# tlemane/kmtricks

Measured on AMD Instinct MI355X. Metric: k-mers merged/s (merge stage, sum over partitions of input records / time), higher is better.
Workload: dtype u64 keys / u32 counts (integer)

## Files before the change

kmtricks_amd/csrc/kmx_api.hip:

```cpp
#include "kmx_host.hpp"

#include <algorithm>
#include <chrono>
#include <cmath>
#include <sys/mman.h>
#include <unordered_map>
#include <mutex>
#include <cstdlib>
#include <cstring>
#include <memory>

using namespace kmx;

static thread_local std::string g_create_err;

void* kmx_ctx::dalloc(size_t bytes)
{
  if (bytes == 0) bytes = 256;
  if (bytes >= (8u << 20)) { size_t p2 = (size_t)1 << 23; while (p2 * 2 <= bytes) p2 *= 2; const size_t q = p2 >> 3; bytes = (bytes + q - 1) / q * q; }
  int best = -1;
  for (size_t i = 0; i < pool.size(); i++)
    if (!pool[i].used && pool[i].bytes >= bytes && pool[i].bytes <= 2 * bytes + (1u << 20) &&
        (best < 0 || pool[i].bytes < pool[best].bytes)) best = (int)i;
  if (best >= 0) { pool[best].used = true; return pool[best].p; }
// ... 494 lines not shown
      u32 rt_max = 0; bool rec_bits = true, any_share = false;
      for (auto& H : R->tasks) { rt_max = std::max(rt_max, H.rt); rec_bits = rec_bits && std::max(H.rec_min, H.share_min) <= 1u; any_share = any_share || H.share_min > 0; }
      const u32 bgrid = std::min(R->n_items, (u32)ctx->n_cu * 2u);
      static const bool two_walks_env = getenv("KMX_BFT_TWO_WALKS") != nullptr;
      if (rec_bits && any_share && !R->bft_two_walks && !two_walks_env && !R->d_rem) {
        u64 per_tile = 0;
        for (auto& H : R->tasks) { const u64 tiles = std::max<u64>(1, ((H.upper - H.lower + 1) + H.rt - 1) / H.rt); per_tile = std::max(per_tile, H.total_recs / tiles); }
        u64 cap = std::max<u64>(4096, per_tile / 4);
        cap = std::min<u64>(cap, ((1ull << 30) / 8) / std::max(1u, bgrid));
        R->rem_cap = (u32)cap;
        R->d_rem = (u64*)ctx->dalloc((size_t)bgrid * cap * 8);
      }
      const bool one_walk = R->d_rem && !R->bft_two_walks;
      bool wide = false;
      for (auto& H : R->tasks) { const double m = (double)H.total_recs / H.N * (double)H.rt / (double)(H.upper - H.lower + 1); wide = wide || m + 2.6 * std::sqrt(m) + 8 > (double)bft_round_records(false); }
      KMX_HIP(ctx, launch_merge_bft(d_tasks, d_items, R->n_items, d_ticket, bgrid, R->max_n, rt_max, rec_bits, wide, one_walk ? R->d_rem : nullptr, R->rem_cap, ctx->stream));
    } else
    KMX_HIP(ctx, launch_merge_bf(mode == KMX_MODE_BFC, d_tasks, d_items, R->n_items, d_ticket, R->grid, R->bf_lds, ctx->stream));
  } else if (R->use_cols) {
    const TaskDev* d_subs = reinterpret_cast<const TaskDev*>(R->d_meta + R->o_subtasks);
    const uint2* d_subitems = reinterpret_cast<const uint2*>(R->d_meta + R->o_subitems);
    const ColsDev* d_cols = reinterpret_cast<const ColsDev*>(R->d_meta + R->o_cols);
    const uint2* d_citems = reinterpret_cast<const uint2*>(R->d_meta + R->o_citems);
    static const bool overlap = getenv("KMX_COLS_PREP_OVERLAP") != nullptr;
    hipStream_t ps = overlap ? ctx->aux : ctx->stream;
    if (!R->ev_pre) KMX_HIP(ctx, hipEventCreateWithFlags(&R->ev_pre, hipEventDisableTiming));
    if (overlap && ctx->stream_shared) {
      KMX_HIP(ctx, hipEventRecord(R->ev_pre, ctx->stream));
      KMX_HIP(ctx, hipStreamWaitEvent(ctx->aux, R->ev_pre, 0));
    }
    if (!overlap) KMX_HIP(ctx, hipStreamWaitEvent(ctx->stream, R->ev_up, 0));
    KMX_HIP(ctx, launch_range_bounds(kw, d_subs, nt, R->sub_max_n, R->sub_max_c, ps));
    KMX_HIP(ctx, CO.skel(d_subs, d_subitems, R->n_subitems, ps));
    KMX_HIP(ctx, CO.prep(d_tasks, d_subs, d_cols, nt, ps));
    {
      u32 max_slots = 0;
      for (auto& H : R->tasks) max_slots = std::max(max_slots, H.slots_cap);
      const char* const tenv = getenv("KMX_COLS_SEED_TRIES");
      KMX_HIP(ctx, CO.seeds(d_tasks, d_cols, nt, max_slots, tenv && atoi(tenv) > 0 ? (u32)atoi(tenv) : 0u, getenv("KMX_TRACE") != nullptr, ps));
    }
    KMX_HIP(ctx, hipEventRecord(R->ev_pre, ps));
    KMX_HIP(ctx, hipStreamWaitEvent(ctx->stream, R->ev_up, 0));
    KMX_HIP(ctx, launch_range_bounds(kw, d_tasks, nt, R->max_n, R->max_c, ctx->stream));
    KMX_HIP(ctx, hipStreamWaitEvent(ctx->stream, R->ev_pre, 0));
    if (R->ev0) KMX_HIP(ctx, hipEventRecord(R->ev0, ctx->stream));
    const u32 cols_grid_env = getenv("KMX_COLS_GRID") ? (u32)atoi(getenv("KMX_COLS_GRID")) : 0u;
    const u32 sparse_cus_env = getenv("KMX_SPARSE_CUS") ? (u32)atoi(getenv("KMX_SPARSE_CUS")) : 0u;
    KMX_HIP(ctx, CO.merge(mode, (R->cols_ext ? 1 : 0) | (R->cols_resc ? 2 : 0) | (R->cols_ord ? 4 : 0) | (R->cols_narrow ? 8 : 0), d_tasks, d_cols, d_citems, R->n_citems, d_ticket,
                          cols_grid_env ? std::min(cols_grid_env, R->cols_grid) : R->cols_grid, ctx->stream));
    if (R->ev0) { if (!R->ev_mid) KMX_HIP(ctx, hipEventCreate(&R->ev_mid)); KMX_HIP(ctx, hipEventRecord(R->ev_mid, ctx->stream)); }
    KMX_HIP(ctx, CO.sparse(mode | (R->cols_resc ? 2 : 0) | (R->cols_ord ? 4 : 0), d_tasks, d_cols, d_items, R->n_items, nt, d_ticket, sparse_cus_env ? std::min(sparse_cus_env, (u32)ctx->n_cu) : (u32)ctx->n_cu, ctx->stream));
    if (R->share_fix) {
      if ((size_t)R->max_n * 4 > 48 * 1024) KMX_HIP(ctx, hipFuncSetAttribute(reinterpret_cast<const void*>(&k_share_fix), hipFuncAttributeMaxDynamicSharedMemorySize, (int)std::min<size_t>((size_t)R->max_n * 4, 160 * 1024)));
      hipLaunchKernelGGL(k_share_fix, dim3((unsigned)ctx->n_cu * 2u, nt), dim3(256), (size_t)R->max_n * 4, ctx->stream, (const TaskDev*)d_tasks, kw);
      KMX_HIP(ctx, hipGetLastError());
    }
    if (R->ev0) KMX_HIP(ctx, hipEventRecord(R->ev1, ctx->stream));
    return mirror_and_mark(R);
  } else {
    if (with_bounds) KMX_HIP(ctx, launch_range_bounds(kw, d_tasks, nt, R->max_n, R->max_c, ctx->stream));
    if (R->ev0) KMX_HIP(ctx, hipEventRecord(R->ev0, ctx->stream));
    if (R->use_pivot) KMX_HIP(ctx, launch_merge_pivot(kw, mode, d_tasks, d_items, R->n_items, d_ticket, R->grid, ctx->stream));
    else if (R->rows_small) KMX_HIP(ctx, launch_merge_rows_s(kw, mode, d_tasks, d_items, R->n_items, d_ticket, R->grid, R->max_n, ctx->stream));
    else KMX_HIP(ctx, launch_merge_rows(kw, mode, d_tasks, d_items, R->n_items, d_ticket, R->grid, R->max_n, ctx->stream));
  }
  if (R->ev0) KMX_HIP(ctx, hipEventRecord(R->ev1, ctx->stream));
  return mirror_and_mark(R);
}

__global__ __launch_bounds__(256)
void k_share_fix(const TaskDev* __restrict__ tasks, u32 kw)
{
  extern __shared__ u32 sm_s[];
  const TaskDev& T = tasks[blockIdx.y];
  if (T.mode != KMX_MODE_COUNT || T.share_min <= max(1u, T.rec_min)) return;
  if (T.ctrl[2] & (u64)(ERR_FALLBACK | ERR_ROWS_OVERFLOW)) return;
  const u64 rows = T.ctrl[0];
// ... 238 lines not shown
    max_n = std::max(max_n, H.N); max_c = std::max(max_c, H.c);
  }
  R->n_items = n_items; R->max_n = max_n; R->max_c = max_c;
  R->grid = std::min(n_items, is_bf ? slots : (u32)ctx->n_cu * (u32)(R->rows_small ? rows_s_wgs_per_cu((int)kw) : rows_wgs_per_cu((int)kw)));
  if (R->use_pivot) R->grid = std::min(n_items, (u32)ctx->n_cu);
  if (R->use_cols) {
    R->subs.resize(n_tasks);
    u32 nsub = 0, ncit = 0;
    for (u32 t = 0; t < n_tasks; t++) {
      const TaskHost& H = R->tasks[t];
      TaskHost& Q = R->subs[t];
      { const u32 S = cols_row_lists(std::max(1u, H.rec_min)); Q.N = std::min<u32>(S ? S : 32u, H.N); }
      Q.kw = kw; Q.mode = mode; Q.rec_min = H.rec_min; Q.share_min = 0;
      Q.len.resize(Q.N);
      u32 piv = 0;
      Q.src.resize(Q.N);
      std::vector<u32> win;
      for (u32 i = 0; i < Q.N; i++) {
        const u32 w0 = (u32)(((u64)i * H.N) / Q.N), w1 = std::max(w0 + 1, (u32)(((u64)(i + 1) * H.N) / Q.N));
        win.clear();
        for (u32 j = w0; j < w1; j++) win.push_back(j);
        std::nth_element(win.begin(), win.begin() + win.size() / 2, win.end(), [&](u32 a, u32 b) { return H.len[a] != H.len[b] ? H.len[a] < H.len[b] : a < b; });
        const u32 src = win[win.size() / 2];
        Q.src[i] = src;
        Q.len[i] = H.len[src]; Q.total_recs += H.len[src];
        if (Q.len[i] > Q.len[piv]) piv = i;
      }
      Q.pivot = (Q.N >= 2 && Q.len[Q.N / 2] > 0) ? Q.N / 2 : piv;
      Q.row_bytes = 8 * kw;
      u32 wl = 0; while (wl < 6 && (Q.N << (wl + 1)) <= (u32)rows_cap((int)kw, Q.N)) wl++;
      Q.wl = wl;
      Q.rows_guess = std::max<u64>(1, std::min<u64>(H.rows_guess, Q.total_recs));
      u64 c = std::min<u64>(2000, std::max<u64>(1, Q.total_recs / 1500));
      c = std::min<u64>(c, std::max<u32>(1, Q.len[Q.pivot]));
      Q.c = (u32)c;
      Q.seg_cap = Q.c;
      Q.out_cap_rows = (u64)Q.c * CO.skel_cap();
      Q.out_bytes = (size_t)(Q.out_cap_rows * Q.row_bytes);
      nsub += Q.c; ncit += H.c * H.nblk;
      R->sub_max_c = std::max(R->sub_max_c, Q.c); R->sub_max_n = std::max(R->sub_max_n, Q.N);
    }
    R->n_subitems = nsub; R->n_citems = ncit;
    R->sub_grid = std::min(nsub, (u32)ctx->n_cu * (u32)rows_wgs_per_cu((int)kw));
    R->cols_grid = std::min(ncit, cols_cus);
  }
  if (is_bf) {
    int lds = 0;
    for (auto& H : R->tasks) lds = std::max(lds, bf_lds_bytes(H.rt, H.row_bytes, H.N));
    R->bf_lds = lds;
  }

  for (auto& H : R->tasks) H.kernel = R->use_cols ? 2 : R->use_pivot ? 1 : 0;
  const bool cols = R->use_cols;
  size_t off = 0;
  R->o_tasks = off; off = align_up(off + sizeof(TaskDev) * n_tasks, 256);
  R->o_items = off; off = align_up(off + sizeof(uint2) * n_items, 256);
  R->o_ticket = off; off += 256;
  R->o_ctrl0 = off;
  for (auto& H : R->tasks) { H.o_ctrl = off; off += 64; }
  off = align_up(off, 256);
  auto lay_lists = [&](TaskHost& H) {
    H.o_recs = off; off = align_up(off + 8ull * H.N, 256);
    H.o_len = off; off = align_up(off + 4ull * H.N, 256);
    H.o_smin = off; off = align_up(off + 4ull * H.N, 256);
    H.o_stats = off; off = align_up(off + 8ull * 6 * H.N, 256);
  };
// ... 1193 lines not shown
```

kmtricks_amd/csrc/kmx_dev.hpp:

```cpp
#pragma once
#include <hip/hip_runtime.h>
#include <stdint.h>

namespace kmx {

typedef unsigned long long u64;
typedef uint32_t u32;
typedef uint16_t u16;
typedef uint8_t u8;
typedef __attribute__((address_space(1))) const u32 gu32;
struct __attribute__((packed, aligned(1))) UDword { u32 v; };
struct __attribute__((packed, aligned(1))) UShort { u16 v; };

struct Seg {
  u32 range;
  u32 seq;
  u64 row_off;
  u32 nrows;
  u32 pad;
};

struct TaskDev {
  const u8* const* recs;
  const u32* len;
// ... 49 lines not shown
#define KMX_CHUNK_BYTES 262144
#endif

enum { ERR_ROWS_OVERFLOW = 1, ERR_SEGS_OVERFLOW = 2, ERR_FALLBACK = 4,
       ERR_DIVERGENT = 8,
       ERR_SLICES = 16,
       ERR_DENSE_CAP = 32 };

template <int KW> struct Key { u64 w[KW]; };

template <int KW> __device__ __forceinline__ bool key_less(const Key<KW>& a, const Key<KW>& b) {
#pragma unroll
  for (int i = KW - 1; i > 0; i--) { if (a.w[i] != b.w[i]) return a.w[i] < b.w[i]; }
  return a.w[0] < b.w[0];
}
template <int KW> __device__ __forceinline__ bool key_eq(const Key<KW>& a, const Key<KW>& b) {
  bool e = a.w[0] == b.w[0];
#pragma unroll
  for (int i = 1; i < KW; i++) e = e && (a.w[i] == b.w[i]);
  return e;
}
template <int KW> __device__ __forceinline__ bool key_le(const Key<KW>& a, const Key<KW>& b) { return !key_less<KW>(b, a); }
template <int KW> __device__ __forceinline__ Key<KW> key_inf() { Key<KW> k; for (int i = 0; i < KW; i++) k.w[i] = ~0ULL; return k; }
template <int KW> __device__ __forceinline__ Key<KW> key_min(const Key<KW>& a, const Key<KW>& b) { return key_less<KW>(b, a) ? b : a; }

template <int KW> __device__ __forceinline__ Key<KW> load_key(const u8* p) {
  const u32* q = reinterpret_cast<const u32*>(p);
  Key<KW> k;
#pragma unroll
  for (int i = 0; i < KW; i++) k.w[i] = (u64)q[2 * i] | ((u64)q[2 * i + 1] << 32);
  return k;
}

template <int KW> __device__ __forceinline__ Key<KW> load_row_key(const u8* p) {
  if ((reinterpret_cast<uintptr_t>(p) & 3u) == 0) return load_key<KW>(p);
  Key<KW> k;
#pragma unroll
  for (int i = 0; i < KW; i++) {
    u64 w = 0;
#pragma unroll
    for (int b = 0; b < 8; b++) w |= (u64)p[8 * i + b] << (8 * b);
    k.w[i] = w;
  }
  return k;
}

__device__ __forceinline__ u64 shfl_xor_u64(u64 v, int m) {
  u32 lo = __shfl_xor((u32)v, m), hi = __shfl_xor((u32)(v >> 32), m);
  return (u64)lo | ((u64)hi << 32);
}
template <int KW> __device__ __forceinline__ Key<KW> wave_min_key(Key<KW> k) {
#pragma unroll
  for (int off = 32; off > 0; off >>= 1) {
    Key<KW> o;
#pragma unroll
    for (int i = 0; i < KW; i++) o.w[i] = shfl_xor_u64(k.w[i], off);
    k = key_min<KW>(k, o);
  }
  return k;
}
template <int M> __device__ __forceinline__ u32 xor_lane_u32(u32 v) {
  static_assert(M == 1 || M == 2 || M == 4 || M == 8 || M == 16 || M == 32, "a power of two below 64");
  if constexpr (M == 1) return (u32)__builtin_amdgcn_mov_dpp((int)v, 0xB1, 0xF, 0xF, true);
  else if constexpr (M == 2) return (u32)__builtin_amdgcn_mov_dpp((int)v, 0x4E, 0xF, 0xF, true);
  else if constexpr (M == 4)
    return (u32)__builtin_amdgcn_mov_dpp(__builtin_amdgcn_mov_dpp((int)v, 0x141, 0xF, 0xF, true), 0x1B, 0xF, 0xF, true);
// ... 13 lines not shown
```

kmtricks_amd/csrc/kmx_host.hpp:

```cpp
#pragma once
#include <hip/hip_runtime.h>
#include <string>
#include <functional>
#include <vector>
#include "kmx_dev.hpp"
#include "skf.hpp"
#include "../../include/kmx.h"

namespace kmx {

int rows_lds_bytes(int kw, u32 n_lists);
int rows_cap(int kw, u32 n_lists);
int rows_wgs_per_cu(int kw);
u32 rows_chunk_rows(u32 row_bytes);
u32 rows_image_bytes(int kw);
hipError_t launch_range_bounds(int kw, const TaskDev* tasks, u32 n_tasks, u32 max_n, u32 max_c, hipStream_t st);
hipError_t launch_merge_rows(int kw, int mode, const TaskDev* tasks, const uint2* items, u32 n_items, u32* ticket,
                             u32 grid_x, u32 max_n, hipStream_t st);
int rows_s_cap(int kw, u32 n_lists);
int rows_s_wgs_per_cu(int kw);
u32 rows_s_image_bytes(int kw);
hipError_t launch_merge_rows_s(int kw, int mode, const TaskDev* tasks, const uint2* items, u32 n_items, u32* ticket, u32 grid_x, u32 max_n, hipStream_t st);
int pivot_lds_bytes(int kw);
u32 pivot_max_lists();
hipError_t launch_merge_pivot(int kw, int mode, const TaskDev* tasks, const uint2* items, u32 n_items, u32* ticket,
                              u32 grid_x, hipStream_t st);
struct ColsOps {
  int (*lds_bytes)();
  u32 (*block_lists)();
  u32 (*wgs_per_cu)();
  u32 (*tile_rows)(u32 nb);
  u64 (*scratch_keys)(u32 slots, u32 nblk);
  u64 (*scratch_counts)(u32 slots, u32 nblk);
  u64 (*ext_entries)(u32 slots, u32 nblk);
  u32 (*skel_cap)();
  hipError_t (*skel)(const TaskDev* subs, const uint2* items, u32 n_items, hipStream_t st);
  hipError_t (*prep)(const TaskDev* tasks, const TaskDev* subs, const ColsDev* cols, u32 n_tasks, hipStream_t st);
  hipError_t (*seeds)(const TaskDev* tasks, const ColsDev* cols, u32 n_tasks, u32 max_slots, u32 max_tries, bool trace, hipStream_t st);
  hipError_t (*merge)(int mode, int ext, const TaskDev* tasks, const ColsDev* cols, const uint2* items, u32 n_items, u32* ticket, u32 grid_x, hipStream_t st);
  hipError_t (*sparse)(int mode, const TaskDev* tasks, const ColsDev* cols, const uint2* range_items, u32 n_items, u32 n_tasks, u32* ticket, u32 n_cu, hipStream_t st);
  u64 (*dir_bytes)(u32 slots);
  u32 (*groups)(u32 slots);
  hipError_t (*offsets)(const ColsDev* cols, u32 task, u64* goff, hipStream_t st);
  hipError_t (*gather)(const TaskDev* tasks, const ColsDev* cols, u32 task, u32 n_groups, const u64* goff, u8* body, hipStream_t st);
  hipError_t (*order)(const TaskDev* tasks, const ColsDev* cols, u32 task, u32 n_groups, const u64* goff, u32* order, hipStream_t st);
  void (*dbg_dump)();
  void (*seeds_dump)();
  void (*phase_prof_dump)();
  u32 key_words;
};
const ColsOps& cols_ops_k1();
const ColsOps& cols_ops_k2();
inline const ColsOps& cols_ops(int kw) { return kw == 2 ? cols_ops_k2() : cols_ops_k1(); }
int bf_lds_bytes(u32 rt, u32 nb, u32 n_lists);
hipError_t launch_range_bounds_bf(const TaskDev* tasks, u32 n_tasks, u32 max_n, u32 max_c, hipStream_t st);
hipError_t launch_merge_bf(int bfc, const TaskDev* tasks, const uint2* items, u32 n_items, u32* ticket,
                           u32 grid_x, int lds, hipStream_t st);
u32 bft_tile_rows(u32 rec_min, u32 share_min);
u32 bft_block_lists();
u32 bft_max_lists();
u32 bft_round_records(bool wide);
u32 bft_fit_rows(u32 max_n, bool bits);
hipError_t launch_merge_bft(const TaskDev* tasks, const uint2* items, u32 n_items, u32* ticket, u32 grid_x, u32 max_n, u32 rt_max, bool rec_bits, bool wide, u64* rem, u32 rem_cap, hipStream_t st);
hipError_t launch_bit_transpose(const u8* in, u8* out, u64 nrows, u64 ncols, hipStream_t st);
u32 filter_tiles(u32 n);
hipError_t launch_filter_match(int kw, const u8* rows, u32 n_rows, u64 irb, const u8* key, u32 n_key, int pa,
                               u32* hit, u32* vec, u8* marks, u32* tile_cnt, hipStream_t st);
hipError_t launch_filter_scan(u32* a, u32 n, hipStream_t st);
hipError_t launch_filter_move(const u8* rows, u32 n_rows, u64 irb, u64 orb, const u32* hit, const u32* vec, const u32* tile_base,
                              u8* out, hipStream_t st);
// ... 195 lines not shown
```

kmtricks_amd/csrc/merge_cols.hip:

```cpp
#include "kmx_host.hpp"
#include <algorithm>
#include <cstdio>
#include <cstring>

#ifndef KMX_CL_KW
#define KMX_CL_KW 1
#endif
#if KMX_CL_KW == 1
#define CLNS cols_k1
#elif KMX_CL_KW == 2
#define CLNS cols_k2
#elif KMX_CL_KW == 3
#define CLNS cols_k3
#else
#define CLNS cols_k4
#endif

namespace kmx { namespace CLNS {

#ifndef KMX_CL_TPB
#define KMX_CL_TPB 1024
#endif
constexpr int CL_TPB = KMX_CL_TPB;
constexpr int CL_WGS = 1024 / CL_TPB;
// ... 122 lines not shown
  }
  tries = max_tries;
  return 0;
}
__device__ __forceinline__ void cl_fill(ClEnt* tab, const CKey (&key)[CL_KPL], const bool (&have)[CL_KPL], u32 lane, u32 mult)
{
#pragma unroll
  for (int x = 0; x < CL_KPL; x++) {
    if (have[x]) {
      ClEnt e; memset(&e, 0, sizeof(e)); ent_set(e, key[x]); e.idx = lane + 64u * x + 1;
      tab[cl_thash(key[x], mult)] = e;
    }
  }
}

}

#ifndef KMX_SK_TPB
#define KMX_SK_TPB 256
#endif
constexpr int SK_TPB = KMX_SK_TPB;
constexpr int SK_CAP = 2048;

__global__ __launch_bounds__(SK_TPB)
void k_cols_skel(const TaskDev* __restrict__ subs, const uint2* __restrict__ items, u32 n_items)
{
  __shared__ CKey ks[SK_CAP];
  __shared__ u32 wsum[SK_TPB / 64];
  const u32 item = blockIdx.x;
  if (item >= n_items) return;
  const TaskDev& S = subs[items[item].x];
  const u32 range = items[item].y, N = S.N, rec_min = max(1u, S.rec_min);
  const u32 tid = threadIdx.x, lane = tid & 63, wave = tid >> 6;
  u32 total = 0;
  for (u32 i = 0; i < N; i++) total += S.bounds[(u64)(range + 1) * N + i] - S.bounds[(u64)range * N + i];
  Seg sg; sg.range = range; sg.seq = 0; sg.row_off = (u64)range * SK_CAP; sg.nrows = 0; sg.pad = 0;
  if (total > (u32)SK_CAP) {
    if (tid == 0) { atomicOr(&S.ctrl[2], (u64)ERR_ROWS_OVERFLOW); S.segs[range] = sg; atomicAdd(&S.ctrl[1], 1ULL); }
    return;
  }
  __shared__ u32 irregular;
  u32 maxn = 1;
  for (u32 i = 0; i < N; i++) maxn = max(maxn, S.bounds[(u64)(range + 1) * N + i] - S.bounds[(u64)range * N + i]);
  u32 L = 1; while (L < maxn) L <<= 1;
  u32 SP = 1; while (SP < N) SP <<= 1;
  const bool runs = (u64)SP * L <= (u64)SK_CAP;
  u32 P = 2;
  if (runs) P = max(2u, SP * L); else while (P < total) P <<= 1;
  if (tid == 0) irregular = 0;
  if (runs) for (u32 t = tid; t < P; t += SK_TPB) ks[t] = ck_inf();
  __syncthreads();
  {
    const u32 tpl = max(1u, (u32)SK_TPB / N);
    for (u32 i = tid / tpl; i < N; i += (u32)SK_TPB / tpl) {
      u32 off = 0;
      if (!runs) for (u32 j = 0; j < i; j++) off += S.bounds[(u64)(range + 1) * N + j] - S.bounds[(u64)range * N + j];
      const u32 lo = S.bounds[(u64)range * N + i], n = S.bounds[(u64)(range + 1) * N + i] - lo, smin = S.soft_min[i];
      const u8* base = S.recs[i] + (u64)lo * RB;
      for (u32 e = tid % tpl; e < n; e += tpl) {
        const u32* rp = reinterpret_cast<const u32*>(base + (u64)e * RB);
        const bool solid = rp[RD - 1] >= smin;
        const CKey key = solid ? ck_load(reinterpret_cast<const u8*>(rp)) : ck_inf();
        if (!runs) ks[off + e] = key;
        else { ks[i * L + ((i & 1u) ? L - 1 - e : e)] = key; if (!solid) irregular = 1; }
      }
    }
  }
  if (!runs) for (u32 t = total + tid; t < P; t += SK_TPB) ks[t] = ck_inf();
  __syncthreads();
  const u32 k0 = (runs && !irregular) ? 2 * L : 2;
  for (u32 k = k0; k <= P; k <<= 1) {
    for (u32 j = k >> 1; j > 0; j >>= 1) {
      for (u32 t = tid; t < P / 2; t += SK_TPB) {
        const u32 a = ((t & ~(j - 1)) << 1) | (t & (j - 1)), b = a | j;
        const CKey x = ks[a], y = ks[b];
        const bool up = (a & k) == 0;
        if (ck_lt(y, x) == up) { ks[a] = y; ks[b] = x; }
      }
      __syncthreads();
    }
  }
  const u32 per = P / SK_TPB ? P / SK_TPB : 1;
  u32 mine = 0, keptm = 0, nsolid = 0, ncov = 0;
  for (u32 x = 0; x < per; x++) {
    const u32 i = tid * per + x;
    if (i < P) {
      const CKey k = ks[i];
      const bool real = !ck_eq(k, ck_inf());
      const bool kept = real && (i == 0 || !ck_eq(ks[i - 1], k)) && i + rec_min - 1 < P && ck_eq(ks[i + rec_min - 1], k);
      keptm |= (kept ? 1u : 0u) << x; mine += kept ? 1u : 0u;
      if (real && (range & 7u) == 0) {
        nsolid++;
        bool cov = false;
        for (u32 j = 0; j < rec_min && !cov; j++) cov = i >= j && i - j + rec_min - 1 < P && ck_eq(ks[i - j], k) && ck_eq(ks[i - j + rec_min - 1], k);
        ncov += cov ? 1u : 0u;
      }
    }
  }
  if ((range & 7u) == 0) {
#pragma unroll
    for (int off = 32; off > 0; off >>= 1) { nsolid += __shfl_xor(nsolid, off); ncov += __shfl_xor(ncov, off); }
    if (lane == 0 && nsolid) { atomicAdd(&S.ctrl[4], (u64)nsolid); atomicAdd(&S.ctrl[5], (u64)ncov); }
  }
  const u32 incl = wave_incl_scan(mine, (int)lane);
  if (lane == 63) wsum[wave] = incl;
  __syncthreads();
  u32 base = incl - mine, nk = 0;
  for (u32 w = 0; w < SK_TPB / 64; w++) { if (w < wave) base += wsum[w]; nk += wsum[w]; }
  CKey* out = reinterpret_cast<CKey*>(S.out) + (u64)range * SK_CAP;
  for (u32 x = 0; x < per; x++) if ((keptm >> x) & 1u) out[base++] = ks[tid * per + x];
  if (tid == 0) { sg.nrows = nk; S.segs[range] = sg; atomicAdd(&S.ctrl[1], 1ULL); atomicAdd(&S.ctrl[3], (u64)nk); }
}

constexpr int CP_TPB = 1024;
__global__ __launch_bounds__(CP_TPB)
void k_cols_prep(const TaskDev* __restrict__ tasks, const TaskDev* __restrict__ subs, const ColsDev* __restrict__ cols)
{
  const TaskDev& T = tasks[blockIdx.x];
  const TaskDev& S = subs[blockIdx.x];
  const ColsDev& C = cols[blockIdx.x];
  __shared__ u32 s_off[CP_MAXSEG];
  __shared__ u64 s_ord[CP_MAXSEG];
  __shared__ u32 s_n[CP_MAXSEG];
  const u32 tid = threadIdx.x;
  const u64 serr = S.ctrl[2], nseg64 = S.ctrl[1], rows = S.ctrl[3];
  if (tid == 0) T.ctrl[7] = rows;
  const u64 slots = rows / C.rt + T.c + 2;
  const bool dense_small = C.dense != nullptr && rows > (u64)C.dense_cap;
  const bool bad = serr != 0 || nseg64 > (u64)CP_MAXSEG || nseg64 > S.seg_cap || rows > T.out_cap_rows || rows > 0xFFFFFF00ULL ||
                   slots > C.slots_cap || dense_small;
  const u64 nsolid = S.ctrl[4], ncov = S.ctrl[5];
  const bool divergent = (nsolid - ncov) * 8 > nsolid;
  if (divergent && !bad) {
    if (tid == 0) { atomicOr(&T.ctrl[2], (u64)(ERR_FALLBACK | ERR_DIVERGENT)); *C.nskel = 0; atomicAdd(&kmx_cols_dbg[4], 1u); }
    for (u32 j = tid; j <= T.c; j += CP_TPB) { C.rbounds[j] = 0; if (C.gbase) C.gbase[j] = 0; }
    return;
  }
  if (bad) {
    const bool only_dense = dense_small && !(serr != 0 || nseg64 > (u64)CP_MAXSEG || nseg64 > S.seg_cap || rows > T.out_cap_rows || rows > 0xFFFFFF00ULL || slots > C.slots_cap);
    if (tid == 0) { atomicOr(&T.ctrl[2], (u64)(ERR_FALLBACK | (only_dense ? ERR_DENSE_CAP : 0))); *C.nskel = 0; }
    for (u32 j = tid; j <= T.c; j += CP_TPB) { C.rbounds[j] = 0; if (C.gbase) C.gbase[j] = 0; }
    return;
  }
  const u32 nseg = (u32)nseg64;
  const u32 srb = S.row_bytes;
  for (u32 i = tid; i < nseg; i += CP_TPB) { const Seg a = S.segs[i]; s_ord[i] = ((u64)a.range << 32) | a.seq; s_n[i] = a.nrows; }
  __syncthreads();
  for (u32 i = tid; i < nseg; i += CP_TPB) {
    const u64 mine = s_ord[i];
    u32 off = 0;
    for (u32 j = 0; j < nseg; j++) off += s_ord[j] < mine ? s_n[j] : 0u;
    s_off[i] = off;
  }
  __syncthreads();
  for (u32 i = tid >> 6; i < nseg; i += CP_TPB / 64) {
    const Seg a = S.segs[i];
    const u8* src = S.out + a.row_off * srb;
    for (u32 r = tid & 63u; r < a.nrows; r += 64) reinterpret_cast<CKey*>(C.skel)[(u64)s_off[i] + r] = ck_load(src + (u64)r * srb);
  }
  __syncthreads();
  const u32 np = T.len[T.pivot];
  for (u32 j = tid; j <= T.c; j += CP_TPB) {
    u32 res;
    if (j == 0) res = 0;
    else if (j == T.c) res = (u32)rows;
    else {
      const u32 pos = (u32)(((u64)j * np) / T.c);
      const CKey q = ck_load(T.recs[T.pivot] + (u64)pos * RB);
      u32 lo = 0, hi = (u32)rows;
      while (lo < hi) { const u32 mid = lo + ((hi - lo) >> 1); if (ck_lt(reinterpret_cast<const CKey*>(C.skel)[mid], q)) lo = mid + 1; else hi = mid; }
      res = lo;
    }
    C.rbounds[j] = res;
  }
  if (tid == 0) {
    *C.nskel = (u32)rows;
    T.ctrl[0] = rows; T.ctrl[1] = 1; T.ctrl[3] = rows;
    Seg sg; sg.range = 0; sg.seq = 0; sg.row_off = 0; sg.nrows = (u32)rows; sg.pad = 0;
    T.segs[0] = sg;
  }
  if (C.gbase) {
    __shared__ u32 s_ng;
    __syncthreads();
    if (tid == 0) {
      u32 g = 0;
      for (u32 j = 0; j < T.c; j++) { C.gbase[j] = g; const u32 n = C.rbounds[j + 1] - C.rbounds[j]; g += max(1u, (n + C.rt - 1) / C.rt) * (u32)CL_HALVES; }
      C.gbase[T.c] = g; s_ng = g;
      atomicMax(C.gmax, g);
    }
    __syncthreads();
    const u32 ng = s_ng;
    for (u32 g = tid; g < ng; g += CP_TPB) {
      u32 lo = 0, hi = T.c;
      while (hi - lo > 1) { const u32 mid = (lo + hi) >> 1; if (C.gbase[mid] <= g) lo = mid; else hi = mid; }
      C.gmap[g] = make_uint4(lo + 1, g - C.gbase[lo], C.rbounds[lo], C.rbounds[lo + 1]);
    }
  }
}

constexpr int CS_TPB = 256;
constexpr u32 CS_TRIES = 1024;
__device__ u32 kmx_cols_tries[12];
__global__ __launch_bounds__(CS_TPB)
void k_cols_seeds(const TaskDev* __restrict__ tasks, const ColsDev* __restrict__ cols, u32 max_tries, u32 trace)
{
  __shared__ u32 bm[CS_TPB / 64][CL_PT / 32];
  __shared__ u32 s_fail;
  const TaskDev& T = tasks[blockIdx.y];
  const ColsDev& C = cols[blockIdx.y];
  const u32 tid = threadIdx.x, lane = tid & 63u, wave = tid >> 6;
  if (tid == 0) s_fail = 0;
  if (__syncthreads_or((__hip_atomic_load(&T.ctrl[2], __ATOMIC_RELAXED, __HIP_MEMORY_SCOPE_AGENT) & (u64)(ERR_FALLBACK | ERR_ROWS_OVERFLOW)) != 0)) return;
  const u32 slot = blockIdx.x * (u32)(CS_TPB / 64) + wave, c = T.c, rt = C.rt;
  if (slot < C.slots_cap && slot <= C.rbounds[c] / rt + c) {
    u32 lo = 0, hi = c;
    while (hi - lo > 1) { const u32 mid = (lo + hi) >> 1; if (C.rbounds[mid] / rt + mid <= slot) lo = mid; else hi = mid; }
    const u32 s_lo = C.rbounds[lo], s_hi = C.rbounds[lo + 1];
    const u32 q = slot - (s_lo / rt + lo), ntiles = max(1u, (s_hi - s_lo + rt - 1) / rt);
    if (q < ntiles) {
      const u32 s0 = s_lo + q * rt;
      CKey key[CL_KPL]; bool have[CL_KPL];
#pragma unroll
      for (int x = 0; x < CL_KPL; x++) {
        const u32 j = lane + 64u * x;
        have[x] = j < rt && s0 + j < s_hi;
        key[x] = have[x] ? reinterpret_cast<const CKey*>(C.skel)[s0 + j] : ck_inf();
      }
      u32 tries = 0;
// ... 1306 lines not shown
void cols_phase_prof_dump()
{
  u64 h[8];
  if (hipMemcpyFromSymbol(h, HIP_SYMBOL(kmx_cols_prof), sizeof(h)) != hipSuccess) return;
  u64 tot = 0; for (int i = 0; i < 8; i++) tot += h[i];
  static const char* nm[8] = {"item setup", "window wait", "scan", "bar(scan)", "tile out", "bar(out)", "-", "-"};
  for (int i = 0; i < 6; i++) fprintf(stderr, "[cols] %-12s %6.2f%%  %llu\n", nm[i], tot ? 100.0 * h[i] / tot : 0.0, h[i]);
  memset(h, 0, sizeof(h));
  (void)hipMemcpyToSymbol(HIP_SYMBOL(kmx_cols_prof), h, sizeof(h));
  if (hipMemcpyFromSymbol(h, HIP_SYMBOL(kmx_sparse_prof), sizeof(h)) != hipSuccess) return;
  tot = 0; for (int i = 0; i < 8; i++) tot += h[i];
  static const char* sn[8] = {"group entries", "zero maps", "mark twice | sample + place", "candidates | rank", "sort", "runs + claim", "rows", "gather (rec-min 1)"};
  for (int i = 0; i < 8; i++) fprintf(stderr, "[sparse] %-14s %6.2f%%  %llu\n", sn[i], tot ? 100.0 * h[i] / tot : 0.0, h[i]);
  memset(h, 0, sizeof(h));
  (void)hipMemcpyToSymbol(HIP_SYMBOL(kmx_sparse_prof), h, sizeof(h));
}
#endif

int cols_lds_bytes() { return CL_IMG + CL_NT * CL_PT * (int)sizeof(ClEnt) + 64 + 256; }
u32 cols_halves() { return CL_HALVES; }
u32 cols_wgs_per_cu() { return CL_WGS; }
u32 cols_block_lists() { return CL_NB; }
u32 cols_tile_rows(u32 nb) { return std::max(1u, std::min<u32>((u32)CL_RT, (u32)CL_IMG / (4u * std::max(1u, nb)))); }
u64 cols_scratch_keys(u32 slots, u32 nblk) { return (u64)slots * CL_HALVES * nblk * CL_NW * CL_OVW * EW; }
u64 cols_scratch_counts(u32 slots, u32 nblk) { return (u64)slots * CL_HALVES * nblk * CL_NW; }
u64 cols_ext_entries(u32 slots, u32 nblk) { return std::max<u64>(64 * 1024, (u64)slots * CL_HALVES * nblk * CL_NW * CL_OVW / 16); }

u32 cols_skel_cap() { return SK_CAP; }
hipError_t launch_cols_skel(const TaskDev* subs, const uint2* items, u32 n_items, hipStream_t st)
{
  hipLaunchKernelGGL(k_cols_skel, dim3(n_items), dim3(SK_TPB), 0, st, subs, items, n_items);
  return hipGetLastError();
}
hipError_t launch_cols_prep(const TaskDev* tasks, const TaskDev* subs, const ColsDev* cols, u32 n_tasks, hipStream_t st)
{
  hipLaunchKernelGGL(k_cols_prep, dim3(n_tasks), dim3(CP_TPB), 0, st, tasks, subs, cols);
  return hipGetLastError();
}
hipError_t launch_cols_seeds(const TaskDev* tasks, const ColsDev* cols, u32 n_tasks, u32 max_slots, u32 max_tries, bool trace, hipStream_t st)
{
  const u32 per = (u32)(CS_TPB / 64);
  hipLaunchKernelGGL(k_cols_seeds, dim3((max_slots + per - 1) / per, n_tasks), dim3(CS_TPB), 0, st, tasks, cols, max_tries ? max_tries : CS_TRIES, trace ? 1u : 0u);
  return hipGetLastError();
}
template <int MODE, bool EXT, bool RESC, bool ORD, bool NAR>
static hipError_t launch_merge_cols_as(const TaskDev* tasks, const ColsDev* cols, const uint2* items, u32 n_items, u32* ticket, u32 grid_x, hipStream_t st)
{
  const int lds = cols_lds_bytes();
  hipError_t e = hipFuncSetAttribute(reinterpret_cast<const void*>(&k_merge_cols<MODE, EXT, RESC, ORD, NAR>), hipFuncAttributeMaxDynamicSharedMemorySize, lds);
  if (e != hipSuccess) return e;
  hipLaunchKernelGGL((k_merge_cols<MODE, EXT, RESC, ORD, NAR>), dim3(grid_x), dim3(CL_TPB), lds, st, tasks, cols, items, n_items, ticket);
  return hipGetLastError();
}
hipError_t launch_merge_cols(int mode, int ext, const TaskDev* tasks, const ColsDev* cols, const uint2* items, u32 n_items, u32* ticket, u32 grid_x, hipStream_t st)
{
  const bool x = ext & 1, r = (ext & 2) != 0, o = (ext & 4) != 0, n = (ext & 8) != 0 && o && mode == 0;
#define KMX_CL_L3(M, X, R) (o ? launch_merge_cols_as<M, X, R, true, false>(tasks, cols, items, n_items, ticket, grid_x, st) : launch_merge_cols_as<M, X, R, false, false>(tasks, cols, items, n_items, ticket, grid_x, st))
#define KMX_CL_LAUNCH(M) (r ? (x ? KMX_CL_L3(M, true, true) : KMX_CL_L3(M, false, true)) : (x ? KMX_CL_L3(M, true, false) : KMX_CL_L3(M, false, false)))
  if (n) return r ? (x ? launch_merge_cols_as<0, true, true, true, true>(tasks, cols, items, n_items, ticket, grid_x, st) : launch_merge_cols_as<0, false, true, true, true>(tasks, cols, items, n_items, ticket, grid_x, st))
                  : (x ? launch_merge_cols_as<0, true, false, true, true>(tasks, cols, items, n_items, ticket, grid_x, st) : launch_merge_cols_as<0, false, false, true, true>(tasks, cols, items, n_items, ticket, grid_x, st));
  return mode == 0 ? KMX_CL_LAUNCH(0) : KMX_CL_LAUNCH(1);
#undef KMX_CL_L3
#undef KMX_CL_LAUNCH
}
template <int MODE, bool RESC>
static hipError_t launch_cols_sparse_ord(const TaskDev* tasks, const ColsDev* cols, u32 n_tasks, u32* ticket, u32 n_cu, hipStream_t st)
{
  static int per_cu = 0;
  if (per_cu == 0) {
// ... 65 lines not shown
```

kmtricks_amd/csrc/merge_rows.hip:

```cpp
#include "kmx_dev.hpp"
#include <algorithm>
#include <cstdio>
#include <cstring>

#ifdef KMX_ROWS_SMALL
#define k_merge_rows k_merge_rows_s
#define cap_of cap_of_s
#define ts_of ts_of_s
#define rows_emit_bytes rows_emit_bytes_s
#define rows_fixed_bytes rows_fixed_bytes_s
#define rows_big rows_big_s
#define rows_lds_bytes rows_s_lds_bytes
#define rows_cap rows_s_cap
#define rows_wgs_per_cu rows_s_wgs_per_cu
#define rows_image_bytes rows_s_image_bytes
#define launch_merge_rows launch_merge_rows_s
#define kmx_phase_prof kmx_phase_prof_s
#define rows_phase_prof_dump rows_s_phase_prof_dump
#endif

namespace kmx {

#ifndef KMX_ROWS_TPB
#define KMX_ROWS_TPB 1024
#endif
#ifndef KMX_ROWS_CAP
#define KMX_ROWS_CAP 4096
#endif
constexpr int TPB = KMX_ROWS_TPB;
constexpr int CAP = KMX_ROWS_CAP;
constexpr int WGS_PER_CU = (TPB <= 512 && (CAP * 8 + 2 * CAP * 4 + CAP * 2 + 4096 + 384) * 2 <= 160 * 1024) ? 2 : 1;
constexpr int NWAVE = TPB / 64;
__host__ __device__ constexpr int cap_of(int kw, bool big = false) { return kw <= 2 || (big && kw == 3) ? CAP : (big && kw == 4) ? 3 * CAP / 4 : CAP / 2; }
__host__ __device__ constexpr int ts_of(int cap) { int t = 1; while (t < 2 * cap) t *= 2; return t; }

__host__ __device__ inline int rows_emit_bytes(int kw, bool big = false) { return cap_of(kw, big) * kw * 8; }
__host__ __device__ inline int rows_fixed_bytes(int kw, bool big = false) { return cap_of(kw, big) * kw * 8 + ts_of(cap_of(kw, big)) * 4 + cap_of(kw, big) * 2 + 4096; }

#ifndef KMX_ROWS_SMALL
template <int KW>
__global__ void k_range_bounds(const TaskDev* __restrict__ tasks, u32 max_c)
{
  const TaskDev& T = tasks[blockIdx.z];
  const u32 i = blockIdx.x * blockDim.x + threadIdx.x;
  const u32 j = blockIdx.y;
  if (i >= T.N || j > T.c) return;
  const u32 n = T.len[i];
  u32 res;
  if (j == 0) res = 0;
  else if (j == T.c) res = n;
  else {
    constexpr int RB = KW * 8 + 4;
    const u32 np = T.len[T.pivot];
    const u32 pos = (u32)(((u64)j * np) / T.c);
    const Key<KW> q = load_key<KW>(T.recs[T.pivot] + (u64)pos * RB);
    const u8* base = T.recs[i];
    u32 lo = 0, hi = n;
    if (n) {
      const u32 g = (u32)min((u64)n - 1, ((u64)pos * n) / np);
      if (key_less<KW>(load_key<KW>(base + (u64)g * RB), q)) {
        lo = g + 1;
        u32 step = 1, pr = g + 1;
        while (pr < n && key_less<KW>(load_key<KW>(base + (u64)pr * RB), q)) { lo = pr + 1; step <<= 1; pr = g + step; }
        hi = min(pr, n);
      } else {
        hi = g;
        u32 step = 1;
        while (step <= g && !key_less<KW>(load_key<KW>(base + (u64)(g - step) * RB), q)) { hi = g - step; step <<= 1; }
        lo = step <= g ? g - step + 1 : 0;
      }
    }
    while (lo < hi) {
      u32 mid = lo + ((hi - lo) >> 1);
      Key<KW> k = load_key<KW>(base + (u64)mid * RB);
      if (key_less<KW>(k, q)) lo = mid + 1; else hi = mid;
    }
    res = lo;
  }
  T.bounds[(u64)j * T.N + i] = res;
}
#endif

#ifdef KMX_PHASE_PROF
__device__ u64 kmx_phase_prof[16];
#endif

template <int KW, int TS> __device__ __forceinline__ u32 key_hash(const Key<KW>& k)
{
  u32 x = (u32)k.w[0] ^ ((u32)(k.w[0] >> 32) * 0x9E3779B1u);
  if (KW >= 2) x ^= ((u32)k.w[KW - 1] * 0x85EBCA77u) ^ ((u32)(k.w[KW - 1] >> 32) * 0xC2B2AE3Du);
  if (KW >= 3) x ^= ((u32)k.w[1] * 0x27D4EB2Fu) ^ ((u32)(k.w[1] >> 32) * 0x165667B1u);
  if (KW >= 4) x ^= ((u32)k.w[2] * 0x9E3779B1u) ^ ((u32)(k.w[2] >> 32) * 0x85EBCA77u);
  x *= 0x85EBCA6Bu; x ^= x >> 15; x *= 0x2C1B3C6Du; x ^= x >> 13;
  return x & (TS - 1);
}

__device__ __forceinline__ void lds_barrier() { asm volatile("s_waitcnt lgkmcnt(0)\n\ts_barrier" ::: "memory"); }

template <int KW, int TS>
__device__ __noinline__ u64 probe_slow(u32* tab, const Key<KW>* keysL, Key<KW> k, u32 h, u32 s)
{
  for (;;) {
    h = (h + 1) & (TS - 1);
    u32 o = tab[h];
    if (o == 0) {
      o = atomicCAS(&tab[h], 0u, s + 1);
      if (o == 0) return (u64)h;
    }
    if (key_eq<KW>(keysL[(o & 0xFFFFu) - 1], k)) return (u64)h | ((u64)o << 32);
  }
}

// ... 437 lines not shown
```

Baseline: 132.2 billion.

## Fuse range-bounds into cols prep kernel and parallelize skeleton searches

When prep overlap is disabled, the per-task range-bounds computation is folded into extra blocks of the cols prep kernel, removing a separate launch and an event sync. The skel kernel computes per-list bounds, offsets and max once per lane using wave scans and shuffles instead of serial loops, and loads four records at a time. The prep kernel batches skeleton copies across two segments with four loads in flight, and replaces per-thread binary searches for cut points with cooperative G-ary searches using ballots. Cut and group tables are kept in LDS when they fit. It also adds an env knob for the sub-range count. Risks include the larger prep grid, and the skel fast path assumes at most 64 lists, falling back to the overflow-error path otherwise.

```diff
diff --git a/kmtricks_amd/csrc/kmx_api.hip b/kmtricks_amd/csrc/kmx_api.hip
--- a/kmtricks_amd/csrc/kmx_api.hip
+++ b/kmtricks_amd/csrc/kmx_api.hip
@@ -550,17 +550,19 @@
     if (!overlap) KMX_HIP(ctx, hipStreamWaitEvent(ctx->stream, R->ev_up, 0));
     KMX_HIP(ctx, launch_range_bounds(kw, d_subs, nt, R->sub_max_n, R->sub_max_c, ps));
     KMX_HIP(ctx, CO.skel(d_subs, d_subitems, R->n_subitems, ps));
-    KMX_HIP(ctx, CO.prep(d_tasks, d_subs, d_cols, nt, ps));
+    KMX_HIP(ctx, CO.prep(d_tasks, d_subs, d_cols, nt, overlap ? 0u : R->max_n, R->max_c, ps));
     {
       u32 max_slots = 0;
       for (auto& H : R->tasks) max_slots = std::max(max_slots, H.slots_cap);
       const char* const tenv = getenv("KMX_COLS_SEED_TRIES");
       KMX_HIP(ctx, CO.seeds(d_tasks, d_cols, nt, max_slots, tenv && atoi(tenv) > 0 ? (u32)atoi(tenv) : 0u, getenv("KMX_TRACE") != nullptr, ps));
     }
-    KMX_HIP(ctx, hipEventRecord(R->ev_pre, ps));
-    KMX_HIP(ctx, hipStreamWaitEvent(ctx->stream, R->ev_up, 0));
-    KMX_HIP(ctx, launch_range_bounds(kw, d_tasks, nt, R->max_n, R->max_c, ctx->stream));
-    KMX_HIP(ctx, hipStreamWaitEvent(ctx->stream, R->ev_pre, 0));
+    if (overlap) {
+      KMX_HIP(ctx, hipEventRecord(R->ev_pre, ps));
+      KMX_HIP(ctx, hipStreamWaitEvent(ctx->stream, R->ev_up, 0));
+      KMX_HIP(ctx, launch_range_bounds(kw, d_tasks, nt, R->max_n, R->max_c, ctx->stream));
+      KMX_HIP(ctx, hipStreamWaitEvent(ctx->stream, R->ev_pre, 0));
+    }
     if (R->ev0) KMX_HIP(ctx, hipEventRecord(R->ev0, ctx->stream));
     const u32 cols_grid_env = getenv("KMX_COLS_GRID") ? (u32)atoi(getenv("KMX_COLS_GRID")) : 0u;
     const u32 sparse_cus_env = getenv("KMX_SPARSE_CUS") ? (u32)atoi(getenv("KMX_SPARSE_CUS")) : 0u;
@@ -865,6 +867,7 @@
       Q.wl = wl;
       Q.rows_guess = std::max<u64>(1, std::min<u64>(H.rows_guess, Q.total_recs));
       u64 c = std::min<u64>(2000, std::max<u64>(1, Q.total_recs / 1500));
+      if (const char* const cenv = getenv("KMX_COLS_SUB_RANGES")) if (atoi(cenv) > 0) c = std::min<u64>((u64)atoi(cenv), 1u << 20);
       c = std::min<u64>(c, std::max<u32>(1, Q.len[Q.pivot]));
       Q.c = (u32)c;
       Q.seg_cap = Q.c;
diff --git a/kmtricks_amd/csrc/kmx_dev.hpp b/kmtricks_amd/csrc/kmx_dev.hpp
--- a/kmtricks_amd/csrc/kmx_dev.hpp
+++ b/kmtricks_amd/csrc/kmx_dev.hpp
@@ -105,6 +105,39 @@
   return k;
 }
 
+template <int KW> __device__ __forceinline__ u32 range_bound(const TaskDev& T, u32 i, u32 j)
+{
+  const u32 n = T.len[i];
+  if (j == 0) return 0;
+  if (j == T.c) return n;
+  constexpr int RB = KW * 8 + 4;
+  const u32 np = T.len[T.pivot];
+  const u32 pos = (u32)(((u64)j * np) / T.c);
+  const Key<KW> q = load_key<KW>(T.recs[T.pivot] + (u64)pos * RB);
+  const u8* base = T.recs[i];
+  u32 lo = 0, hi = n;
+  if (n) {
+    const u32 g = (u32)min((u64)n - 1, ((u64)pos * n) / np);
+    if (key_less<KW>(load_key<KW>(base + (u64)g * RB), q)) {
+      lo = g + 1;
+      u32 step = 1, pr = g + 1;
+      while (pr < n && key_less<KW>(load_key<KW>(base + (u64)pr * RB), q)) { lo = pr + 1; step <<= 1; pr = g + step; }
+      hi = min(pr, n);
+    } else {
+      hi = g;
+      u32 step = 1;
+      while (step <= g && !key_less<KW>(load_key<KW>(base + (u64)(g - step) * RB), q)) { hi = g - step; step <<= 1; }
+      lo = step <= g ? g - step + 1 : 0;
+    }
+  }
+  while (lo < hi) {
+    u32 mid = lo + ((hi - lo) >> 1);
+    Key<KW> k = load_key<KW>(base + (u64)mid * RB);
+    if (key_less<KW>(k, q)) lo = mid + 1; else hi = mid;
+  }
+  return lo;
+}
+
 template <int KW> __device__ __forceinline__ Key<KW> load_row_key(const u8* p) {
   if ((reinterpret_cast<uintptr_t>(p) & 3u) == 0) return load_key<KW>(p);
   Key<KW> k;
diff --git a/kmtricks_amd/csrc/kmx_host.hpp b/kmtricks_amd/csrc/kmx_host.hpp
--- a/kmtricks_amd/csrc/kmx_host.hpp
+++ b/kmtricks_amd/csrc/kmx_host.hpp
@@ -14,8 +14,7 @@
 int rows_wgs_per_cu(int kw);
 u32 rows_chunk_rows(u32 row_bytes);
 u32 rows_image_bytes(int kw);
-hipError_t launch_range_bounds(int kw, const TaskDev* tasks, u32 n_tasks, u32 max_n, u32 max_c, hipStream_t st);
-hipError_t launch_merge_rows(int kw, int mode, const TaskDev* tasks, const uint2* items, u32 n_items, u32* ticket,
+hipError_t launch_range_bounds(int kw, const TaskDev* tasks, u32 n_tasks, u32 max_n, u32 max_c, hipStream_t st);hipError_t launch_merge_rows(int kw, int mode, const TaskDev* tasks, const uint2* items, u32 n_items, u32* ticket,
                              u32 grid_x, u32 max_n, hipStream_t st);
 int rows_s_cap(int kw, u32 n_lists);
 int rows_s_wgs_per_cu(int kw);
@@ -35,7 +34,7 @@
   u64 (*ext_entries)(u32 slots, u32 nblk);
   u32 (*skel_cap)();
   hipError_t (*skel)(const TaskDev* subs, const uint2* items, u32 n_items, hipStream_t st);
-  hipError_t (*prep)(const TaskDev* tasks, const TaskDev* subs, const ColsDev* cols, u32 n_tasks, hipStream_t st);
+  hipError_t (*prep)(const TaskDev* tasks, const TaskDev* subs, const ColsDev* cols, u32 n_tasks, u32 bounds_max_n, u32 bounds_max_c, hipStream_t st);
   hipError_t (*seeds)(const TaskDev* tasks, const ColsDev* cols, u32 n_tasks, u32 max_slots, u32 max_tries, bool trace, hipStream_t st);
   hipError_t (*merge)(int mode, int ext, const TaskDev* tasks, const ColsDev* cols, const uint2* items, u32 n_items, u32* ticket, u32 grid_x, hipStream_t st);
   hipError_t (*sparse)(int mode, const TaskDev* tasks, const ColsDev* cols, const uint2* range_items, u32 n_items, u32 n_tasks, u32* ticket, u32 n_cu, hipStream_t st);
diff --git a/kmtricks_amd/csrc/merge_cols.hip b/kmtricks_amd/csrc/merge_cols.hip
--- a/kmtricks_amd/csrc/merge_cols.hip
+++ b/kmtricks_amd/csrc/merge_cols.hip
@@ -178,16 +178,22 @@
   const TaskDev& S = subs[items[item].x];
   const u32 range = items[item].y, N = S.N, rec_min = max(1u, S.rec_min);
   const u32 tid = threadIdx.x, lane = tid & 63, wave = tid >> 6;
-  u32 total = 0;
-  for (u32 i = 0; i < N; i++) total += S.bounds[(u64)(range + 1) * N + i] - S.bounds[(u64)range * N + i];
+  u32 my_lo = 0, my_n = 0, my_smin = 0; u64 my_recs = 0;
+  if (lane < N) {
+    my_lo = S.bounds[(u64)range * N + lane]; my_n = S.bounds[(u64)(range + 1) * N + lane] - my_lo;
+    my_smin = S.soft_min[lane]; my_recs = (u64)reinterpret_cast<uintptr_t>(S.recs[lane]);
+  }
+  const u32 my_off = wave_incl_scan(my_n, (int)lane) - my_n;
+  u32 total = (u32)__shfl((int)(my_off + my_n), 63), maxn = max(1u, my_n);
+#pragma unroll
+  for (int o = 32; o > 0; o >>= 1) maxn = max(maxn, (u32)__shfl_xor((int)maxn, o));
+  if (N > 64u) total = (u32)SK_CAP + 1;
   Seg sg; sg.range = range; sg.seq = 0; sg.row_off = (u64)range * SK_CAP; sg.nrows = 0; sg.pad = 0;
   if (total > (u32)SK_CAP) {
     if (tid == 0) { atomicOr(&S.ctrl[2], (u64)ERR_ROWS_OVERFLOW); S.segs[range] = sg; atomicAdd(&S.ctrl[1], 1ULL); }
     return;
   }
   __shared__ u32 irregular;
-  u32 maxn = 1;
-  for (u32 i = 0; i < N; i++) maxn = max(maxn, S.bounds[(u64)(range + 1) * N + i] - S.bounds[(u64)range * N + i]);
   u32 L = 1; while (L < maxn) L <<= 1;
   u32 SP = 1; while (SP < N) SP <<= 1;
   const bool runs = (u64)SP * L <= (u64)SK_CAP;
@@ -198,17 +204,30 @@
   __syncthreads();
   {
     const u32 tpl = max(1u, (u32)SK_TPB / N);
-    for (u32 i = tid / tpl; i < N; i += (u32)SK_TPB / tpl) {
-      u32 off = 0;
-      if (!runs) for (u32 j = 0; j < i; j++) off += S.bounds[(u64)(range + 1) * N + j] - S.bounds[(u64)range * N + j];
-      const u32 lo = S.bounds[(u64)range * N + i], n = S.bounds[(u64)(range + 1) * N + i] - lo, smin = S.soft_min[i];
-      const u8* base = S.recs[i] + (u64)lo * RB;
-      for (u32 e = tid % tpl; e < n; e += tpl) {
-        const u32* rp = reinterpret_cast<const u32*>(base + (u64)e * RB);
-        const bool solid = rp[RD - 1] >= smin;
-        const CKey key = solid ? ck_load(reinterpret_cast<const u8*>(rp)) : ck_inf();
-        if (!runs) ks[off + e] = key;
-        else { ks[i * L + ((i & 1u) ? L - 1 - e : e)] = key; if (!solid) irregular = 1; }
+    for (u32 i0 = 0; i0 < N; i0 += (u32)SK_TPB / tpl) {
+      const u32 i = i0 + tid / tpl;
+      const int src = (int)min(i, 63u);
+      const u32 off = (u32)__shfl((int)my_off, src), lo = (u32)__shfl((int)my_lo, src), smin = (u32)__shfl((int)my_smin, src);
+      const u32 n = i < N ? (u32)__shfl((int)my_n, src) : 0u;
+      const u64 recs = (u64)(u32)__shfl((int)(u32)my_recs, src) | ((u64)(u32)__shfl((int)(u32)(my_recs >> 32), src) << 32);
+      const u8* base = reinterpret_cast<const u8*>((uintptr_t)recs) + (u64)lo * RB;
+      for (u32 e0 = tid % tpl; e0 < n; e0 += 4u * tpl) {
+        CKey k4[4]; u32 c4[4];
+#pragma unroll
+        for (u32 x = 0; x < 4u; x++) {
+          const u32 e = e0 + x * tpl;
+          if (e < n) { const u32* rp = reinterpret_cast<const u32*>(base + (u64)e * RB); c4[x] = rp[RD - 1]; k4[x] = ck_load(reinterpret_cast<const u8*>(rp)); }
+        }
+#pragma unroll
+        for (u32 x = 0; x < 4u; x++) {
+          const u32 e = e0 + x * tpl;
+          if (e < n) {
+            const bool solid = c4[x] >= smin;
+            const CKey key = solid ? k4[x] : ck_inf();
+            if (!runs) ks[off + e] = key;
+            else { ks[i * L + ((i & 1u) ? L - 1 - e : e)] = key; if (!solid) irregular = 1; }
+          }
+        }
       }
     }
   }
@@ -260,14 +279,22 @@
 
 constexpr int CP_TPB = 1024;
 __global__ __launch_bounds__(CP_TPB)
-void k_cols_prep(const TaskDev* __restrict__ tasks, const TaskDev* __restrict__ subs, const ColsDev* __restrict__ cols)
-{
+void k_cols_prep(const TaskDev* __restrict__ tasks, const TaskDev* __restrict__ subs, const ColsDev* __restrict__ cols, u32 n_tasks, u32 bx, u32 by)
+{
+  if (blockIdx.x >= n_tasks) {
+    const u32 blk = blockIdx.x - n_tasks;
+    const TaskDev& B = tasks[blk / (bx * by)];
+    const u32 i = (blk % bx) * (u32)CP_TPB + threadIdx.x, j = (blk / bx) % by;
+    if (i < B.N && j <= B.c) B.bounds[(u64)j * B.N + i] = range_bound<KW>(B, i, j);
+    return;
+  }
   const TaskDev& T = tasks[blockIdx.x];
   const TaskDev& S = subs[blockIdx.x];
   const ColsDev& C = cols[blockIdx.x];
   __shared__ u32 s_off[CP_MAXSEG];
   __shared__ u64 s_ord[CP_MAXSEG];
   __shared__ u32 s_n[CP_MAXSEG];
+  __shared__ u64 s_row[CP_MAXSEG];
   const u32 tid = threadIdx.x;
   const u64 serr = S.ctrl[2], nseg64 = S.ctrl[1], rows = S.ctrl[3];
   if (tid == 0) T.ctrl[7] = rows;
@@ -289,8 +316,14 @@
     return;
   }
   const u32 nseg = (u32)nseg64;
-  const u32 srb = S.row_bytes;
-  for (u32 i = tid; i < nseg; i += CP_TPB) { const Seg a = S.segs[i]; s_ord[i] = ((u64)a.range << 32) | a.seq; s_n[i] = a.nrows; }
+  const u32 srb = S.row_bytes, c = T.c, lane = tid & 63u;
+  u32 G = 64; while (G > 1 && (u64)G * (c > 1 ? c - 1 : 1) > (u64)CP_TPB) G >>= 1;
+  const u32 ngroups = (u32)CP_TPB / G, grp = tid / G, gl = tid % G;
+  const u32 np = T.len[T.pivot];
+  const u8* const precs = T.recs[T.pivot];
+  CKey q1 = ck_inf();
+  if (1 + grp < c) q1 = ck_load(precs + (u64)(u32)(((u64)(1 + grp) * np) / c) * RB);
+  for (u32 i = tid; i < nseg; i += CP_TPB) { const Seg a = S.segs[i]; s_ord[i] = ((u64)a.range << 32) | a.seq; s_n[i] = a.nrows; s_row[i] = a.row_off; }
   __syncthreads();
   for (u32 i = tid; i < nseg; i += CP_TPB) {
     const u64 mine = s_ord[i];
@@ -299,47 +332,79 @@
     s_off[i] = off;
   }
   __syncthreads();
-  for (u32 i = tid >> 6; i < nseg; i += CP_TPB / 64) {
-    const Seg a = S.segs[i];
-    const u8* src = S.out + a.row_off * srb;
-    for (u32 r = tid & 63u; r < a.nrows; r += 64) reinterpret_cast<CKey*>(C.skel)[(u64)s_off[i] + r] = ck_load(src + (u64)r * srb);
+  CKey* const skel = reinterpret_cast<CKey*>(C.skel);
+  constexpr u32 NW = (u32)CP_TPB / 64u;
+  for (u32 i0 = tid >> 6; i0 < nseg; i0 += 2u * NW) {
+    for (u32 r0 = 0;; r0 += 256u) {
+      CKey k[2][4];
+      bool more = false;
+#pragma unroll
+      for (u32 s = 0; s < 2u; s++) {
+        const u32 i = i0 + s * NW, n = i < nseg ? s_n[i] : 0u;
+        const u8* src = S.out + s_row[min(i, (u32)CP_MAXSEG - 1u)] * srb;
+#pragma unroll
+        for (u32 x = 0; x < 4u; x++) { const u32 r = r0 + 64u * x + lane; if (r < n) k[s][x] = ck_load(src + (u64)r * srb); }
+        more = more || r0 + 256u < n;
+      }
+#pragma unroll
+      for (u32 s = 0; s < 2u; s++) {
+        const u32 i = i0 + s * NW, n = i < nseg ? s_n[i] : 0u;
+        const u64 off = s_off[min(i, (u32)CP_MAXSEG - 1u)];
+#pragma unroll
+        for (u32 x = 0; x < 4u; x++) { const u32 r = r0 + 64u * x + lane; if (r < n) skel[off + r] = k[s][x]; }
+      }
+      if (!more) break;
+    }
   }
   __syncthreads();
-  const u32 np = T.len[T.pivot];
-  for (u32 j = tid; j <= T.c; j += CP_TPB) {
-    u32 res;
-    if (j == 0) res = 0;
-    else if (j == T.c) res = (u32)rows;
-    else {
-      const u32 pos = (u32)(((u64)j * np) / T.c);
-      const CKey q = ck_load(T.recs[T.pivot] + (u64)pos * RB);
-      u32 lo = 0, hi = (u32)rows;
-      while (lo < hi) { const u32 mid = lo + ((hi - lo) >> 1); if (ck_lt(reinterpret_cast<const CKey*>(C.skel)[mid], q)) lo = mid + 1; else hi = mid; }
-      res = lo;
-    }
-    C.rbounds[j] = res;
+  const bool cuts_in_lds = (u64)c + 1 <= (u64)CP_MAXSEG;
+  u32* const sr = cuts_in_lds ? reinterpret_cast<u32*>(s_ord) : C.rbounds;
+  u32* const sg = cuts_in_lds ? reinterpret_cast<u32*>(s_ord) + CP_MAXSEG : C.gbase;
+  for (u32 jb = 1; jb < c; jb += ngroups) {
+    const u32 j = jb + grp;
+    const bool mine = j < c;
+    CKey q = q1;
+    if (jb != 1u && mine) q = ck_load(precs + (u64)(u32)(((u64)j * np) / c) * RB);
+    u32 lo = 0, hi = mine ? (u32)rows : 0u;
+    const u32 shift = lane & ~(G - 1u);
+    const u64 gmask = G == 64u ? ~0ULL : ((1ULL << G) - 1ULL);
+    while (__ballot(lo < hi) != 0ULL) {
+      const u32 n = hi - lo;
+      const bool below = lo < hi && ck_lt(skel[lo + (u32)(((u64)(gl + 1u) * n) / (G + 1u))], q);
+      const u32 f = (u32)__popcll((__ballot(below) >> shift) & gmask);
+      if (lo < hi) {
+        const u32 nlo = f ? lo + (u32)(((u64)f * n) / (G + 1u)) + 1u : lo;
+        hi = f < G ? lo + (u32)(((u64)(f + 1u) * n) / (G + 1u)) : hi;
+        lo = nlo;
+      }
+    }
+    if (mine && gl == 0) { sr[j] = lo; if (cuts_in_lds) C.rbounds[j] = lo; }
   }
   if (tid == 0) {
+    sr[0] = 0; sr[c] = (u32)rows;
+    if (cuts_in_lds) { C.rbounds[0] = 0; C.rbounds[c] = (u32)rows; }
     *C.nskel = (u32)rows;
     T.ctrl[0] = rows; T.ctrl[1] = 1; T.ctrl[3] = rows;
-    Seg sg; sg.range = 0; sg.seq = 0; sg.row_off = 0; sg.nrows = (u32)rows; sg.pad = 0;
-    T.segs[0] = sg;
+    Seg all; all.range = 0; all.seq = 0; all.row_off = 0; all.nrows = (u32)rows; all.pad = 0;
+    T.segs[0] = all;
   }
   if (C.gbase) {
     __shared__ u32 s_ng;
     __syncthreads();
+    const u32 rt = C.rt;
     if (tid == 0) {
       u32 g = 0;
-      for (u32 j = 0; j < T.c; j++) { C.gbase[j] = g; const u32 n = C.rbounds[j + 1] - C.rbounds[j]; g += max(1u, (n + C.rt - 1) / C.rt) * (u32)CL_HALVES; }
-      C.gbase[T.c] = g; s_ng = g;
+      for (u32 j = 0; j < c; j++) { sg[j] = g; const u32 n = sr[j + 1] - sr[j]; g += max(1u, (n + rt - 1) / rt) * (u32)CL_HALVES; }
+      sg[c] = g; s_ng = g;
       atomicMax(C.gmax, g);
     }
     __syncthreads();
     const u32 ng = s_ng;
+    if (cuts_in_lds) for (u32 j = tid; j <= c; j += CP_TPB) C.gbase[j] = sg[j];
     for (u32 g = tid; g < ng; g += CP_TPB) {
-      u32 lo = 0, hi = T.c;
-      while (hi - lo > 1) { const u32 mid = (lo + hi) >> 1; if (C.gbase[mid] <= g) lo = mid; else hi = mid; }
-      C.gmap[g] = make_uint4(lo + 1, g - C.gbase[lo], C.rbounds[lo], C.rbounds[lo + 1]);
+      u32 lo = 0, hi = c;
+      while (hi - lo > 1) { const u32 mid = (lo + hi) >> 1; if (sg[mid] <= g) lo = mid; else hi = mid; }
+      C.gmap[g] = make_uint4(lo + 1, g - sg[lo], sr[lo], sr[lo + 1]);
     }
   }
 }
@@ -1712,9 +1777,12 @@
   hipLaunchKernelGGL(k_cols_skel, dim3(n_items), dim3(SK_TPB), 0, st, subs, items, n_items);
   return hipGetLastError();
 }
-hipError_t launch_cols_prep(const TaskDev* tasks, const TaskDev* subs, const ColsDev* cols, u32 n_tasks, hipStream_t st)
-{
-  hipLaunchKernelGGL(k_cols_prep, dim3(n_tasks), dim3(CP_TPB), 0, st, tasks, subs, cols);
+hipError_t launch_cols_prep(const TaskDev* tasks, const TaskDev* subs, const ColsDev* cols, u32 n_tasks, u32 bounds_max_n, u32 bounds_max_c, hipStream_t st)
+{
+  const u32 bx = bounds_max_n ? (bounds_max_n + (u32)CP_TPB - 1) / (u32)CP_TPB : 0u, by = bounds_max_c + 1;
+  const u64 blocks = (u64)n_tasks + (u64)bx * by * n_tasks;
+  if (blocks > 0x7FFFFFFFULL) return hipErrorInvalidValue;
+  hipLaunchKernelGGL(k_cols_prep, dim3((u32)blocks), dim3(CP_TPB), 0, st, tasks, subs, cols, n_tasks, bx, by);
   return hipGetLastError();
 }
 hipError_t launch_cols_seeds(const TaskDev* tasks, const ColsDev* cols, u32 n_tasks, u32 max_slots, u32 max_tries, bool trace, hipStream_t st)
diff --git a/kmtricks_amd/csrc/merge_rows.hip b/kmtricks_amd/csrc/merge_rows.hip
--- a/kmtricks_amd/csrc/merge_rows.hip
+++ b/kmtricks_amd/csrc/merge_rows.hip
@@ -45,39 +45,7 @@
   const u32 i = blockIdx.x * blockDim.x + threadIdx.x;
   const u32 j = blockIdx.y;
   if (i >= T.N || j > T.c) return;
-  const u32 n = T.len[i];
-  u32 res;
-  if (j == 0) res = 0;
-  else if (j == T.c) res = n;
-  else {
-    constexpr int RB = KW * 8 + 4;
-    const u32 np = T.len[T.pivot];
-    const u32 pos = (u32)(((u64)j * np) / T.c);
-    const Key<KW> q = load_key<KW>(T.recs[T.pivot] + (u64)pos * RB);
-    const u8* base = T.recs[i];
-    u32 lo = 0, hi = n;
-    if (n) {
-      const u32 g = (u32)min((u64)n - 1, ((u64)pos * n) / np);
-      if (key_less<KW>(load_key<KW>(base + (u64)g * RB), q)) {
-        lo = g + 1;
-        u32 step = 1, pr = g + 1;
-        while (pr < n && key_less<KW>(load_key<KW>(base + (u64)pr * RB), q)) { lo = pr + 1; step <<= 1; pr = g + step; }
-        hi = min(pr, n);
-      } else {
-        hi = g;
-        u32 step = 1;
-        while (step <= g && !key_less<KW>(load_key<KW>(base + (u64)(g - step) * RB), q)) { hi = g - step; step <<= 1; }
-        lo = step <= g ? g - step + 1 : 0;
-      }
-    }
-    while (lo < hi) {
-      u32 mid = lo + ((hi - lo) >> 1);
-      Key<KW> k = load_key<KW>(base + (u64)mid * RB);
-      if (key_less<KW>(k, q)) lo = mid + 1; else hi = mid;
-    }
-    res = lo;
-  }
-  T.bounds[(u64)j * T.N + i] = res;
+  T.bounds[(u64)j * T.N + i] = range_bound<KW>(T, i, j);
 }
 #endif
 
```

After: 128.3 billion. -2.9%, worse.
